# Ogeon/pyrite

Measured on AMD Instinct MI355X. Metric: Msamples/sec, higher is better.
Workload: dtype f32; 1 GPU; C3: c3_mesh_in_box, 1920x1080, 1024 spp; bounces=8, light_samples=4, spectrum_samples=10, spectrum_bins=64, tile_size=32, triangles=819212, spheres=0, parallelism=one launch on one GPU, film_weight_check=ok

## Files before the change

### pyrite_amd/csrc/api.cpp

```cpp
#include <hip/hip_runtime.h>

#include <algorithm>
#include <chrono>
#include <cmath>
#include <cstdlib>
#include <cstring>
#include <memory>
#include <new>
#include <string>
#include <vector>

#include "api_internal.h"
#include "bvh.h"
#include "bvh_device.h"
#include "device_scene.h"
#include "kernels/refit_launch.h"
#include "program_regs.h"

using namespace pyr;

namespace {

thread_local std::string g_error;
int fail(int code, const std::string& message) {
// ... 277 lines not shown
        if (!closed) return false;
    }
    chain.assign(outer_first.rbegin(), outer_first.rend());
    for (uint32_t reg : chain)
        if (reg >= PYR_MAX_NUMBER_REGISTERS) return false;
    hit = lambda = p;
    hit.first_instr = (uint32_t)instrs.size();
    hit.num_instrs = (uint32_t)hit_list.size();
    hit.output_reg = chain[0];
    instrs.insert(instrs.end(), hit_list.begin(), hit_list.end());
    lambda.first_instr = (uint32_t)instrs.size();
    lambda.num_instrs = (uint32_t)lambda_list.size();
    lambda.output_reg = instrs[(size_t)lambda_writer].output;
    instrs.insert(instrs.end(), lambda_list.begin(), lambda_list.end());
    return true;
}

}

struct PyrScene {
    int device = 0;
    int num_cus = 0;
    DevScene dev{};
    PyrBvhInfo info{};
    PyrBuildInfo build_info{};
    std::unique_ptr<pyr::BuiltBvh> digest_source;
    DeviceBuffer wide_nodes, wide_pair_nodes, pair_prims, nodes, prims, tri_shade, spheres, sphere_material, planes, plane_material, lamps, materials, components, programs, instrs, spectra,
        spectrum_data, rgb_basis, counters, tri_tex, sphere_tex_scale, plane_frames, textures, texture_data;
    PyrCounters last_counters{};
    bool have_counters = false;
    PyrProgramInfo program_info{};
    uint32_t* tail_count = nullptr;
    DeviceBuffer tape;
    DeviceBuffer tape_overflow;
    struct Geometry {
        std::vector<float> tri_positions, tri_normals, tri_uvs, tri_frames, spheres, sphere_tex_scale;
        std::vector<uint32_t> tri_material, sphere_material;
        std::vector<PyrLamp> lamps;
        bool has_uvs = false, has_frames = false, has_tex_scale = false;
        uint32_t num_triangles = 0, num_spheres = 0;
        PyrSceneDesc view() const {
            PyrSceneDesc d{};
            d.num_triangles = num_triangles, d.num_spheres = num_spheres, d.num_lamps = (uint32_t)lamps.size();
            d.tri_positions = tri_positions.data(), d.tri_normals = tri_normals.data(), d.tri_material = tri_material.data();
            d.tri_uvs = has_uvs ? tri_uvs.data() : nullptr, d.tri_frames = has_frames ? tri_frames.data() : nullptr;
            d.spheres = spheres.data(), d.sphere_material = sphere_material.data();
            d.sphere_tex_scale = has_tex_scale ? sphere_tex_scale.data() : nullptr;
            d.lamps = lamps.data();
            return d;
        }
    } geometry;
    void keep_geometry(const PyrSceneDesc* d) {
        Geometry& g = geometry;
        const size_t nt = d->num_triangles, ns = d->num_spheres;
        g.num_triangles = d->num_triangles, g.num_spheres = d->num_spheres;
        g.tri_positions.assign(d->tri_positions, d->tri_positions + (nt ? 9 * nt : 0));
        g.tri_normals.assign(d->tri_normals, d->tri_normals + (nt ? 9 * nt : 0));
        g.tri_material.assign(d->tri_material, d->tri_material + nt);
        g.has_uvs = d->tri_uvs != nullptr, g.has_frames = d->tri_frames != nullptr, g.has_tex_scale = d->sphere_tex_scale != nullptr;
        if (g.has_uvs) g.tri_uvs.assign(d->tri_uvs, d->tri_uvs + 6 * nt);
        if (g.has_frames) g.tri_frames.assign(d->tri_frames, d->tri_frames + 12 * nt);
        g.spheres.assign(d->spheres, d->spheres + (ns ? 4 * ns : 0));
        g.sphere_material.assign(d->sphere_material, d->sphere_material + ns);
        if (g.has_tex_scale) g.sphere_tex_scale.assign(d->sphere_tex_scale, d->sphere_tex_scale + 2 * ns);
        g.lamps.assign(d->lamps, d->lamps + d->num_lamps);
    }
// ... 513 lines not shown
    const uint32_t rows = p->film_row_count ? p->film_row_count : film->height;
    return (uint64_t)rows * film->width * film->bins;
}

int check_render_args(PyrScene* scene, const PyrCamera* camera, const PyrFilmDesc* film, const PyrRenderParams* p, const void* film_ptr) {
    if (!scene || !camera || !film || !p || !film_ptr) return fail(PYR_ERR_INVALID_ARGUMENT, "null argument");
    if (film->width == 0 || film->height == 0 || film->bins == 0 || p->tile_size == 0 || p->spectrum_samples == 0)
        return fail(PYR_ERR_INVALID_ARGUMENT, "zero-sized parameter");
    if (!(film->wl_width > 0.0f)) return fail(PYR_ERR_INVALID_ARGUMENT, "empty wavelength span");
    uint32_t rows = p->film_row_count ? p->film_row_count : film->height;
    if ((uint64_t)p->film_row_begin + rows > film->height) return fail(PYR_ERR_INVALID_ARGUMENT, "film window exceeds the image");
    if (p->spectrum_samples > 64) return fail(PYR_ERR_UNSUPPORTED, "spectrum_samples > 64");
    if ((uint64_t)film->width * film->height >= 0xFFFFFFFFull) return fail(PYR_ERR_UNSUPPORTED, "image too large: 2^32 pixels or more");
    if (p->film_layout == PYR_FILM_TILE_BLOCKS) {
        const uint64_t tiles = (uint64_t)((film->width + p->tile_size - 1) / p->tile_size) * ((film->height + p->tile_size - 1) / p->tile_size);
        if (tiles * (p->tile_size + 2ull) * (p->tile_size + 2ull) >= 0xFFFFFFFFull) return fail(PYR_ERR_UNSUPPORTED, "image too large for a film of tile blocks");
    }
    if (p->film_layout > PYR_FILM_TILE_BLOCKS) return fail(PYR_ERR_INVALID_ARGUMENT, "unknown film layout");
    if (p->film_layout == PYR_FILM_TILE_BLOCKS && (p->film_row_begin || p->film_row_count))
        return fail(PYR_ERR_INVALID_ARGUMENT, "a film of tile blocks has no row window");
    return PYR_OK;
}


int reserve_tape(PyrScene* scene, RenderLaunch& L, hipStream_t stream) {
    const size_t bytes = (size_t)L.tape_lanes * L.tape_max_ops * sizeof(unsigned long long);
    if (bytes > scene->tape.bytes) {
        HIP_TRY(hipStreamSynchronize(stream));
        scene->tape.release();
        int rc = scene->tape.alloc(bytes);
        if (rc != PYR_OK) return rc;
    }
    L.tape = (unsigned long long*)scene->tape.ptr;
    if (!scene->tape_overflow.ptr) {
        int rc = scene->tape_overflow.alloc(sizeof(uint32_t));
        if (rc != PYR_OK) return rc;
        HIP_TRY(hipMemsetAsync(scene->tape_overflow.ptr, 0, sizeof(uint32_t), stream));
    }
    L.tape_overflow = (uint32_t*)scene->tape_overflow.ptr;
    return PYR_OK;
}

void choose_schedule(const PyrScene* scene, RenderLaunch& L) {
    const char* e = std::getenv("PYRITE_SCHEDULER");
    if (e && std::string(e) == "sm")
        L.scheduler = 1;
    else if (e && std::string(e) == "sync")
        L.scheduler = 0;
    else
        L.scheduler = scene_is_lds_resident(scene->dev) && scene->dev.needs_interpreter == 0 ? 0u : 1u;
    if (L.scheduler == 0 && scene->dev.needs_interpreter != 0) L.scheduler = 1;
    const char* lanes = std::getenv("PYRITE_SM_LANES");
    const char* steps = std::getenv("PYRITE_SM_STEPS");
    L.sm_phase_lanes = lanes && *lanes ? (uint32_t)std::strtoul(lanes, nullptr, 10) : (scene->dev.needs_interpreter != 0 ? 32u : 16u);
    L.sm_trav_steps = steps && *steps ? (uint32_t)std::strtoul(steps, nullptr, 10) : 8u;
    const char* expose = std::getenv("PYRITE_SM_EXPOSE_LANES");
    L.sm_expose_lanes = expose && *expose ? (uint32_t)std::strtoul(expose, nullptr, 10) : L.sm_phase_lanes;
}

int render_batches(PyrScene* scene, RenderLaunch L, bool count, hipStream_t stream) {
    if (L.chunk_end == L.chunk_begin) return PYR_OK;
    choose_schedule(scene, L);
    if (L.scheduler != 0 && (scene->dev.needs_interpreter == 0 || uses_hit_tape(scene->dev, L))) {
        L.tape_lanes = tape_lanes_bound(scene->num_cus);
        L.tape_max_ops = tape_ops_bound(scene->dev, L);
        int rc = reserve_tape(scene, L, stream);
// ... 1350 lines not shown
```

### pyrite_amd/csrc/device_scene.h

```cpp
#pragma once
#include <cstddef>
#include <cstdint>

#include "../../include/pyrite_gpu.h"

namespace pyr {

struct DevPrim {
    float a[4], b[4], c[4];
};

struct DevPrimPair {
    float q[5][4];
};

struct DevTriShade {
    float n1[4], n2[4], n3[4];
};

struct DevTriTex {
    float uv12[4], uv3[4], f1[4], f2[4], f3[4];
};

struct DevTexture {
// ... 86 lines not shown
constexpr uint32_t tape_row(uint32_t slot) { return slot + (slot >= kTapeOneRow ? 1u : 0u); }
constexpr uint32_t tape_rgb_row(uint32_t n_spectral) { return n_spectral + 3u <= kTapeOneRow ? n_spectral : (n_spectral >= kTapeOneRow ? n_spectral + 1u : kTapeValueRows); }
constexpr uint32_t tape_rows_needed(uint32_t n_spectral, bool rgb) {
    return (rgb ? tape_rgb_row(n_spectral) + 3u : (n_spectral == 0u ? 0u : tape_row(n_spectral - 1u) + 1u)) > kTapeValueRows
               ? (rgb ? tape_rgb_row(n_spectral) + 3u : tape_row(n_spectral - 1u) + 1u)
               : kTapeValueRows;
}

constexpr uint32_t kMaxStackDepth = 64;

struct RenderLaunch {
    PyrCamera camera;
    PyrFilmDesc film;
    uint32_t bounces, light_samples, spectrum_samples, tile_size, pixel_samples;
    uint32_t tiles_x, tiles_y;
    uint32_t tile_begin, tile_stride, tile_count;
    uint32_t chunks_per_tile;
    uint32_t chunk_begin, chunk_end;
    uint32_t film_layout;
    uint32_t film_row_begin, film_row_count;
    uint64_t seed;
    float grains_per_wavelength;
    PyrGrain* film_out;
    unsigned long long* counters;
    uint32_t scheduler;
    uint32_t sm_phase_lanes, sm_trav_steps;
    uint32_t sm_expose_lanes;
    uint32_t stack_lds;
    unsigned long long* tape;
    uint32_t tape_lanes, tape_max_ops;
    uint32_t* tape_overflow;
    uint32_t tape_programs_lds;
    uint32_t sample_begin;
};

constexpr uint32_t kFeedSegments = 8, kFeedCursorStride = 64;
constexpr size_t kFeedBytes = (size_t)kFeedSegments * kFeedCursorStride * sizeof(uint32_t);

struct IntersectLaunch {
    const float* rays;
    PyrHit* hits;
    uint32_t n;
    unsigned long long* counters;
    uint32_t* next;
    uint32_t num_cus;
    uint32_t reserve;
    uint32_t stack_lds;
};

struct DevelopLaunch {
    PyrFilmDesc film;
    const PyrGrain* grains;
    float step_size, xyz_scale;
    uint32_t sample_count;
    const float* filter;
    const float* white_div;
    const float* white_mul;
    const float* xyz_table;
    uint32_t xyz_count;
    float xyz_min, xyz_max;
    uint8_t* rgb_out;
    const PyrGrain* grains_b;
};
int launch_develop(const DevelopLaunch& launch, void* stream);

constexpr uint32_t kWaveDevelopMaxBins = 255;
bool develop_wave_serves(const DevelopLaunch& launch);
// ... 83 lines not shown
```

### pyrite_amd/csrc/kernels.hip

```cpp
#ifndef PYRITE_KERNELS_HIP
#define PYRITE_KERNELS_HIP
#include <hip/hip_runtime.h>

#include <algorithm>
#include <cstdint>
#include <cstdlib>
#include <string>
#include <type_traits>

#include "device_scene.h"
#include "exact_math.h"

#ifdef PYR_WIDE_VM
#define PYR_VM_NUMBERS PYR_WIDE_NUMBER_REGISTERS
#define PYR_VM_VECTORS PYR_WIDE_VECTOR_REGISTERS
#define PYR_VM_RGBS PYR_WIDE_RGB_REGISTERS
#else
#define PYR_VM_NUMBERS PYR_MAX_NUMBER_REGISTERS
#define PYR_VM_VECTORS PYR_MAX_VECTOR_REGISTERS
#define PYR_VM_RGBS PYR_MAX_RGB_REGISTERS
#endif
static_assert((PYR_VM_NUMBERS & (PYR_VM_NUMBERS - 1)) == 0 && (PYR_VM_VECTORS & (PYR_VM_VECTORS - 1)) == 0 && (PYR_VM_RGBS & (PYR_VM_RGBS - 1)) == 0,
              "the interpreter masks register indices: its files are powers of two");

// ... 753 lines not shown
    float from_x, from_y, size_x, size_y;
};
DEV TileArea to_view_area(uint32_t x, uint32_t y, uint32_t w, uint32_t h, uint32_t width, uint32_t height) {
    float iw = (float)width, ih = (float)height;
    float half_max = __fmul_rn(fmaxf(iw, ih), 0.5f);
    TileArea a;
    a.from_x = __fdiv_rn(__fadd_rn((float)x, -__fmul_rn(iw, 0.5f)), half_max);
    a.from_y = __fdiv_rn(__fadd_rn((float)y, -__fmul_rn(ih, 0.5f)), half_max);
    a.size_x = __fdiv_rn((float)w, half_max);
    a.size_y = __fdiv_rn((float)h, half_max);
    return a;
}
DEV f3 transform_point(const float* m, f3 p) {
    float x = m[0] * p.x + m[4] * p.y + m[8] * p.z + m[12];
    float y = m[1] * p.x + m[5] * p.y + m[9] * p.z + m[13];
    float z = m[2] * p.x + m[6] * p.y + m[10] * p.z + m[14];
    float w = m[3] * p.x + m[7] * p.y + m[11] * p.z + m[15];
    float inv = 1.0f / w;
    return mk(x * inv, y * inv, z * inv);
}
DEV f3 transform_vector(const float* m, f3 v) {
    return mk(m[0] * v.x + m[4] * v.y + m[8] * v.z, m[1] * v.x + m[5] * v.y + m[9] * v.z, m[2] * v.x + m[6] * v.y + m[10] * v.z);
}
DEV uint32_t f32_as_index(float f) { return f > 0.0f ? (f >= 4294967040.0f ? 0xFFFFFFFFu : (uint32_t)f) : 0u; }

struct Spectral {
    float* base;
    uint32_t s;
    DEV float& wl(uint32_t k) { return base[(0 * s + k) * BLOCK]; }
    DEV float& bright(uint32_t k) { return base[(1 * s + k) * BLOCK]; }
    DEV float& refl(uint32_t k) { return base[(2 * s + k) * BLOCK]; }
};

DEV void surface_at(const DevScene& S, const Hit& hit, f3 o, f3 d, f3& position, f3& normal, uint32_t& material) {
    const uint32_t kind = hit.shape >> 30, index = hit.shape & 0x3FFFFFFFu;
    if (kind == PYR_SHAPE_TRIANGLE) {
        const float4* sh = reinterpret_cast<const float4*>(S.tri_shade) + 3 * (size_t)index;
        const float4 a = sh[0], b = sh[1], c = sh[2];
        float w = 1.0f - (hit.u + hit.v);
        normal = normalize(mk(a.x, a.y, a.z) * w + mk(b.x, b.y, b.z) * hit.u + mk(c.x, c.y, c.z) * hit.v);
        material = __float_as_uint(a.w);
        position = o + d * hit.t;
    } else if (kind == PYR_SHAPE_SPHERE) {
        const float4 sp = reinterpret_cast<const float4*>(S.spheres)[index];
        float dist;
        sphere_test(mk(sp.x, sp.y, sp.z), sp.w, o, d, dist, position);
        normal = normalize(position - mk(sp.x, sp.y, sp.z));
        material = S.sphere_material[index];
    } else {
        const float* pl = S.planes + 8 * index;
        float dist;
        plane_test(ld3(pl), ld3(pl + 3), o, d, dist, position);
        normal = ld3(pl + 3);
        material = S.plane_material[index];
    }
}

struct Quat {
    float s, x, y, z;
};
DEV Quat quat_scale(Quat q, float f) { return Quat{q.s * f, q.x * f, q.y * f, q.z * f}; }
DEV Quat quat_add(Quat a, Quat b) { return Quat{a.s + b.s, a.x + b.x, a.y + b.y, a.z + b.z}; }
DEV Quat quat_normalize(Quat q) {
    float m = sqrt32(q.s * q.s + q.x * q.x + q.y * q.y + q.z * q.z);
    return quat_scale(q, 1.0f / m);
}
// ... 259 lines not shown
DEV void expose_grain(const RenderLaunch& L, uint32_t pixel, float wavelength, float brightness, Counters& cnt) {
    if (pixel == PIXEL_NONE) return;
    uint32_t grain = f32_as_index(__fmul_rn(__fsub_rn(wavelength, L.film.wl_start), L.grains_per_wavelength));
    grain = grain < L.film.bins - 1 ? grain : L.film.bins - 1;
    float* g = reinterpret_cast<float*>(L.film_out + ((size_t)pixel * L.film.bins + grain));
    atomicAdd(g, brightness);
    atomicAdd(g + 1, 1.0f);
    if (COUNT) cnt.exposures++;
}

struct Path {
    Rng rng;
    uint32_t pixel;
    f3 o, d;
    float wl, bright, refl;
    uint32_t bounce, events;
    bool use_additional, sample_light;
};

struct SceneView {
    const float4* nodes;
    const float4* prims;
    bool wide = false;
    const float4* pairs = nullptr;
};
DEV SceneView wide_or_binary_view(const DevScene& S);
template <typename T>
DEV const T* own_scalar(const T* p) {
    unsigned long long in = (unsigned long long)p, out;
    asm volatile("s_mov_b64 %0, %1" : "=s"(out) : "s"(in));
    return reinterpret_cast<const T*>(out);
}

DEV SceneView wide_or_binary_view(const DevScene& S) {
    SceneView v{reinterpret_cast<const float4*>(S.nodes), reinterpret_cast<const float4*>(S.prims), false, nullptr};
    if (S.wide_nodes != nullptr) {
        v.nodes = reinterpret_cast<const float4*>(S.wide_nodes);
        v.wide = true;
    }
    return v;
}

template <bool LDS_SCENE>
DEV SceneView stage_scene(const DevScene& S, float* lds, uint32_t lds_floats_before, bool resumable = false) {
    SceneView v{reinterpret_cast<const float4*>(S.nodes), reinterpret_cast<const float4*>(S.prims)};
    if (!LDS_SCENE && resumable && S.wide_nodes != nullptr) {
        v.nodes = reinterpret_cast<const float4*>(S.wide_nodes);
        v.wide = true;
    }
    if (!LDS_SCENE && resumable && S.wide_nodes != nullptr && S.pair_prims != nullptr) {
        v.nodes = reinterpret_cast<const float4*>(S.wide_pair_nodes);
        v.pairs = reinterpret_cast<const float4*>(S.pair_prims);
    }
    if constexpr (!LDS_SCENE) {
        v.nodes = own_scalar(v.nodes);
        v.prims = own_scalar(v.prims);
        v.pairs = own_scalar(v.pairs);
    }
    if constexpr (LDS_SCENE) {
        float4* staged = reinterpret_cast<float4*>(lds + lds_floats_before);
        const uint32_t node_vecs = S.num_nodes * 4, prim_vecs = S.num_prims * 3;
        for (uint32_t i = threadIdx.x; i < node_vecs; i += BLOCK) staged[i] = v.nodes[i];
        for (uint32_t i = threadIdx.x; i < prim_vecs; i += BLOCK) staged[node_vecs + i] = v.prims[i];
        __syncthreads();
        v.nodes = staged;
        v.prims = staged + node_vecs;
    }
    return v;
}

template <int TABLES, bool COPY = true>
DEV DevScene stage_tables(const DevScene& S, float* lds, uint32_t lds_floats_before) {
    DevScene local = S;
    if (TABLES == 1 || (TABLES == -1 && S.lds_table_floats != 0)) {
        float* dst = lds + lds_floats_before;
        auto stage = [&](const void* src, uint32_t floats) {
            const float* from = reinterpret_cast<const float*>(src);
            if (COPY)
                for (uint32_t i = threadIdx.x; i < floats; i += BLOCK) dst[i] = from[i];
            float* at = dst;
            dst += floats;
            return at;
        };
        local.spectra = reinterpret_cast<const PyrSpectrum*>(stage(S.spectra, S.num_spectra * (uint32_t)(sizeof(PyrSpectrum) / sizeof(float))));
        local.spectrum_data = stage(S.spectrum_data, S.num_spectrum_floats);
        local.materials = reinterpret_cast<const PyrMaterial*>(stage(S.materials, S.num_materials * (uint32_t)(sizeof(PyrMaterial) / sizeof(float))));
        local.components = reinterpret_cast<const PyrComponent*>(stage(S.components, S.num_components * (uint32_t)(sizeof(PyrComponent) / sizeof(float))));
        local.programs = reinterpret_cast<const DevProgram*>(stage(S.programs, S.num_programs * (uint32_t)(sizeof(DevProgram) / sizeof(float))));
        local.lamps = reinterpret_cast<const DevLamp*>(stage(S.lamps, S.num_lamps * (uint32_t)(sizeof(DevLamp) / sizeof(float))));
        if (COPY) __syncthreads();
    }
    return local;
}

template <bool COMPANION_STATE = true>
DEV void start_sample(const RenderLaunch& L, uint32_t tile, uint64_t iteration, const TileArea& area, Path& p, Spectral& spec) {
    const uint32_t SS = L.spectrum_samples;
    p.rng = rng_seed(L.seed, tile, iteration);
    const float px = __fadd_rn(area.from_x, __fmul_rn(area.size_x, rng_f32(p.rng)));
    const float py = __fadd_rn(area.from_y, __fmul_rn(area.size_y, rng_f32(p.rng)));
    p.pixel = film_pixel(L, tile, px, py);
    {
        float focus_x = px / L.camera.view_plane * L.camera.focus_distance;
        float focus_y = py / L.camera.view_plane * L.camera.focus_distance;
        f3 target = mk(focus_x, -focus_y, -L.camera.focus_distance);
        f3 origin = mk(0, 0, 0), direction = target;
        if (L.camera.aperture > 0.0f) {
            float sqrt_r = sqrt32(L.camera.aperture * rng_f32(p.rng));
            float psi = PI_F * 2.0f * rng_f32(p.rng);
            origin = mk(sqrt_r * cos32(psi), sqrt_r * sin32(psi), 0.0f);
            direction = target - origin;
        }
        p.o = transform_point(L.camera.cam_to_world, origin);
        p.d = transform_vector(L.camera.cam_to_world, normalize(direction));
    }
    {
        float step_size = L.film.wl_width / (float)SS;
        float from = L.film.wl_start;
        for (uint32_t k = 0; k < SS; ++k) {
            float to = __fadd_rn(from, step_size);
            spec.wl(k) = rng_range_f32(p.rng, from, to);
            from = to;
        }
        uint32_t hero = rng_range_usize(p.rng, SS);
        p.wl = spec.wl(hero);
        spec.wl(hero) = spec.wl(SS - 1);
        if constexpr (COMPANION_STATE)
            for (uint32_t k = 0; k + 1 < SS; ++k) {
                spec.bright(k) = 0.0f;
// ... 275 lines not shown
    for (uint32_t chunk = L.chunk_begin + wave; chunk < L.chunk_end; chunk += total_waves) {
        uint32_t tile;
        uint64_t iteration;
        TileArea area;
        if (!locate_chunk(L, chunk, lane, tile, iteration, area)) continue;
        Path p{};
        start_sample(launch_from_kernarg(L), tile, iteration, area, p, spec);
        if (COUNT) cnt.samples++;
        SLAP(sp, 0);
        while (p.bounce < L.bounces) {
            const bool ended = bounce_step<COUNT>(S, launch_from_kernarg(L), view, p, spec, stack, cnt, sp);
            p.bounce++;
            if (ended) break;
        }
        SLAP(sp, 6);
        SYNC_PRIO(SYNC_PRIO_E);
        finish_path<COUNT>(launch_from_kernarg(L), p, spec, cnt);
        SLAP(sp, 7);
    }
#ifdef PYR_PHASE_PROFILE
    if (lane == 0)
        for (int i = 0; i < 8; ++i) atomicAdd(&g_phase_prof[i], sp.section[i]);
#endif
    flush_counters<COUNT>(cnt, L.counters);
}

#ifdef PYR_PHASE_PROFILE
#define PROF_DECL unsigned long long prof_c[4] = {0, 0, 0, 0}, prof_l[4] = {0, 0, 0, 0}, prof_n[4] = {0, 0, 0, 0}
#define PROF_BEGIN(ph, cond) const unsigned long long prof_t0_##ph = clock64(); prof_l[ph] += __popcll(ballot64(cond)); prof_n[ph]++
#define PROF_END(ph) prof_c[ph] += clock64() - prof_t0_##ph
#define PROF_LANES(ph, cond) prof_l[ph] += __popcll(ballot64(cond)); prof_n[ph]++
#define PROF_NOW() clock64()
#define PROF_EXTRA(idx, cycles) if ((threadIdx.x & 63u) == 0) atomicAdd(&g_phase_prof[idx], (unsigned long long)(cycles))
#define PROF_FLUSH()                                                                                  \
    if ((threadIdx.x & 63u) == 0)                                                                     \
        for (int i = 0; i < 4; ++i) {                                                                 \
            atomicAdd(&g_phase_prof[i], prof_c[i]);                                                   \
            atomicAdd(&g_phase_prof[4 + i], prof_l[i]);                                               \
            atomicAdd(&g_phase_prof[8 + i], prof_n[i]);                                               \
        }
#else
#define PROF_DECL
#define PROF_BEGIN(ph, cond)
#define PROF_END(ph)
#define PROF_LANES(ph, cond)
#define PROF_NOW() 0ull
#define PROF_EXTRA(idx, cycles)
#define PROF_FLUSH()
#endif

enum Stage : uint32_t { ST_NEW = 0, ST_TRAV = 1, ST_SHADE = 2, ST_NEE = 3, ST_EXPOSE = 4, ST_DONE = 5 };

struct Trav {
    f3 o, d, inv;
    uint32_t nx = 0, ny = 0, nz = 0;
    float limit, closest;
    int node, sp;
    uint32_t shape;
    float u, v;
    bool shadow, blocked;
};

DEV void trav_ray_signs(Trav& t) {
    t.nx = (__float_as_uint(t.d.x) >> 31) * 48u;
    t.ny = (__float_as_uint(t.d.y) >> 31) * 48u;
    t.nz = (__float_as_uint(t.d.z) >> 31) * 48u;
}
DEV float shadow_cutoff(float limit, float margin) { return __builtin_amdgcn_sqrtf(limit * margin + 1.0e-3f); }
DEV void trav_restart(Trav& t, float shadow_margin) {
    if (t.shadow) t.closest = shadow_cutoff(t.limit, shadow_margin);
    t.blocked = false;
    t.node = 0;
    t.sp = 0;
}

template <bool COUNT>
DEV bool trav_begin(const DevScene& S, Trav& t, f3 o, f3 d, bool shadow, float limit, Counters& cnt) {
    t.o = o;
    t.d = d;
    t.shadow = shadow;
    t.blocked = false;
    t.limit = shadow ? limit : -PYR_INF;
    t.closest = PYR_INF;
    t.shape = PYR_HIT_NONE;
    t.u = t.v = 0.0f;
    for (uint32_t i = 0; i < S.num_planes; ++i) {
        const float* pl = S.planes + 8 * i;
        float dist;
        f3 point;
        if (COUNT) cnt.plane_tests++;
        if (plane_test(ld3(pl), ld3(pl + 3), o, d, dist, point)) {
            if (shadow) {
                if (dist > DIST_EPSILON && dist * dist < limit) {
                    t.blocked = true;
                    return true;
                }
            } else if (dist > DIST_EPSILON && dist < t.closest) {
                t.closest = dist;
                t.shape = ((uint32_t)PYR_SHAPE_PLANE << 30) | i;
            }
        }
    }
    trav_restart(t, S.shadow_margin);
    return false;
}

typedef __attribute__((address_space(3))) int lds_int;
struct TravStack {
    lds_int* lds;
    int lds_entries;
    int* deep;
    DEV void push(int sp, int value) {
        if (sp < lds_entries)
            lds[sp * BLOCK] = value;
        else
            deep[sp - lds_entries] = value;
    }
    DEV int pop(int sp) const { return sp < lds_entries ? lds[sp * BLOCK] : deep[sp - lds_entries]; }
};

template <bool COUNT, bool SIGNED = false>
DEV void wide_node_children(const float4 lx, const float4 ly, const float4 lz, const float4 hx, const float4 hy, const float4 hz, const float4 ch, const Trav& t,
                            Counters& cnt, float (&e)[4], int (&c)[4]) {
    const f2v ix = {t.inv.x, t.inv.x}, iy = {t.inv.y, t.inv.y}, iz = {t.inv.z, t.inv.z};
    const float ox = -(t.o.x * t.inv.x), oy = -(t.o.y * t.inv.y), oz = -(t.o.z * t.inv.z);
    const f2v nox = {ox, ox}, noy = {oy, oy}, noz = {oz, oz};
    c[0] = __float_as_int(ch.x), c[1] = __float_as_int(ch.y), c[2] = __float_as_int(ch.z), c[3] = __float_as_int(ch.w);
    {
        const f2v alx = __builtin_elementwise_fma((f2v){lx.x, lx.y}, ix, nox), ahx = __builtin_elementwise_fma((f2v){hx.x, hx.y}, ix, nox);
        const f2v aly = __builtin_elementwise_fma((f2v){ly.x, ly.y}, iy, noy), ahy = __builtin_elementwise_fma((f2v){hy.x, hy.y}, iy, noy);
        const f2v alz = __builtin_elementwise_fma((f2v){lz.x, lz.y}, iz, noz), ahz = __builtin_elementwise_fma((f2v){hz.x, hz.y}, iz, noz);
        const f2v blx = __builtin_elementwise_fma((f2v){lx.z, lx.w}, ix, nox), bhx = __builtin_elementwise_fma((f2v){hx.z, hx.w}, ix, nox);
        const f2v bly = __builtin_elementwise_fma((f2v){ly.z, ly.w}, iy, noy), bhy = __builtin_elementwise_fma((f2v){hy.z, hy.w}, iy, noy);
        const f2v blz = __builtin_elementwise_fma((f2v){lz.z, lz.w}, iz, noz), bhz = __builtin_elementwise_fma((f2v){hz.z, hz.w}, iz, noz);
        const float tl[4][3] = {{alx.x, aly.x, alz.x}, {alx.y, aly.y, alz.y}, {blx.x, bly.x, blz.x}, {blx.y, bly.y, blz.y}};
        const float th[4][3] = {{ahx.x, ahy.x, ahz.x}, {ahx.y, ahy.y, ahz.y}, {bhx.x, bhy.x, bhz.x}, {bhx.y, bhy.y, bhz.y}};
        for (int k = 0; k < 4; ++k) {
            const float tmin = SIGNED ? fmaxf(fmaxf(tl[k][0], tl[k][1]), tl[k][2])
                                      : fmaxf(fmaxf(fminf(tl[k][0], th[k][0]), fminf(tl[k][1], th[k][1])), fminf(tl[k][2], th[k][2]));
            const float tmax = SIGNED ? fminf(fminf(th[k][0], th[k][1]), th[k][2])
// ... 274 lines not shown
struct Walker {
    uint32_t stage = ST_NEW;
    uint32_t n_ops = 0;
    uint32_t tape_column = 0;
    const uint32_t* tape_prepared = nullptr;
    DEV void tape_push(const RenderLaunch& L, uint32_t kind, uint32_t program, float s, bool hero_only = false) {
        if (n_ops < L.tape_max_ops) {
            uint32_t word = (kind << 30) | (hero_only ? TAPE_HERO_ONLY : 0u) | (program & TAPE_PROGRAM_MASK);
            if (tape_prepared != nullptr) {
                uint32_t slot = kTapeOneSlot;
                if (kind != TAPE_SCALE) {
                    const uint32_t* e = tape_prepared + 8 * program;
                    if (e[0] == 0u)
                        s = __uint_as_float(e[1]) * s;
                    else
                        slot = e[7];
                }
                word = (kind == TAPE_ADD ? TAPE_EAGER_ADD : 0u) | (hero_only ? TAPE_HERO_ONLY : 0u) | (slot << TAPE_EAGER_SLOT_SHIFT);
            }
            L.tape[tape_index(n_ops, L.tape_lanes, tape_column)] = (unsigned long long)word | ((unsigned long long)__float_as_uint(s) << 32);
        } else {
            *L.tape_overflow = 1u;
        }
        n_ops++;
    }
    DEV void tape_push_raw(const RenderLaunch& L, uint32_t word, float s) {
        if (n_ops < L.tape_max_ops)
            L.tape[tape_index(n_ops, L.tape_lanes, tape_column)] = (unsigned long long)word | ((unsigned long long)__float_as_uint(s) << 32);
        else
            *L.tape_overflow = 1u;
        n_ops++;
    }
    uint32_t rgb_slot = 0;
    uint32_t chunk = 0;
    Path p{};
    Trav t{};
    f3 b_position = mk(0, 0, 0), b_normal = mk(0, 0, 0), b_out = mk(0, 0, 0);
    bool b_flip = false;
    DEV f3 b_nff() const { return b_flip ? -b_normal : b_normal; }
    bool b_has_brdf = false;
    uint32_t nee_lamp = 0, nee_i = 0;
    DEV static float nee_probability(const DevScene& S, const RenderLaunch& L) {
        const float lamp_probability = 1.0f / (float)S.num_lamps;
        return 1.0f / ((float)L.light_samples * 2.0f * PI_F * lamp_probability);
    }
    bool ls_pending = false, ls_physical = false;
    uint32_t ls_material = 0, ls_color = 0;
    f3 ls_normal = mk(0, 0, 0);
    float ls_scale = 0.0f;
    float ls_tx = 0.0f, ls_ty = 0.0f;

    enum : uint32_t { CONTRIB_NONE = 0, CONTRIB_MUL = 1, CONTRIB_ADD = 2 };
    uint32_t c_kind = CONTRIB_NONE, c_color = 0;
    int c_probability = -1;
    float c_cp = 1.0f, c_outer = 1.0f, c_scale = 1.0f;
    bool c_use_outer = false, c_companions = false, c_has_scale = false;
    f3 c_normal = mk(0, 0, 0), c_incident = mk(0, 0, 0);
    float c_tx = 0.0f, c_ty = 0.0f;
    DEV void contribution(uint32_t kind, uint32_t color, int probability, float cp, bool use_outer, float outer, bool companions, f3 normal, f3 incident, float tx,
                          float ty) {
        c_kind = kind, c_color = color, c_probability = probability, c_cp = cp, c_use_outer = use_outer, c_outer = outer, c_companions = companions;
        c_normal = normal, c_incident = incident, c_tx = tx, c_ty = ty;
    }
    DEV void contribution_clear() {
        c_kind = CONTRIB_NONE, c_color = 0u, c_probability = -1;
        c_cp = 1.0f, c_outer = 1.0f, c_scale = 1.0f;
        c_use_outer = false, c_companions = false, c_has_scale = false;
// ... 109 lines not shown
    }

    DEV void finish_bounce(const DevScene& S, const RenderLaunch& L, Spectral& spec, Counters& cnt) {
        const uint32_t n_add = L.spectrum_samples - 1;
        if (b_has_brdf) {
            const float brdf = 2.0f * fabsf(dot(b_out, b_normal));
            if constexpr (TAPE && !INTERP) {
                tape_push(L, TAPE_SCALE, 0u, brdf);
            } else if constexpr (INTERP) {
                c_scale = brdf, c_has_scale = true;
            } else {
                p.refl *= brdf;
                if (p.use_additional) {
                    for (uint32_t k = 0; k < n_add; ++k) spec.refl(k) *= brdf;
                }
            }
        }
        p.o = b_position;
        p.d = b_out;
        p.bounce++;
        if (p.bounce >= L.bounces) {
            stage = ST_EXPOSE;
        } else {
            if (COUNT) cnt.extension_rays++;
            stage = trav_begin<COUNT>(S, t, p.o, p.d, false, 0.0f, cnt) ? ST_SHADE : ST_TRAV;
        }
    }

    DEV void expose_and_restart(const DevScene& S, const RenderLaunch& L, Spectral& spec, Counters& cnt, uint32_t lane, uint32_t total_waves) {
        if (stage == ST_EXPOSE) {
            if constexpr (!TAPE) finish_path<COUNT>(L, p, spec, cnt);
            stage = ST_NEW;
        }
        if (stage == ST_NEW) {
            stage = ST_DONE;
            while (chunk < L.chunk_end) {
                uint32_t tile;
                uint64_t iteration;
                TileArea area;
                const bool ok = locate_chunk(L, chunk, lane, tile, iteration, area);
                chunk += total_waves;
                if (ok) {
                    start_sample<!TAPE>(L, tile, iteration, area, p, spec);
                    n_ops = 0;
                    if (COUNT) cnt.samples++;
                    if (L.bounces == 0) {
                        stage = ST_EXPOSE;
                    } else {
                        if (COUNT) cnt.extension_rays++;
                        stage = trav_begin<COUNT>(S, t, p.o, p.d, false, 0.0f, cnt) ? ST_SHADE : ST_TRAV;
                    }
                    break;
                }
            }
        }
    }

    DEV void shade(const DevScene& S, const RenderLaunch& L, Spectral& spec, Counters& cnt) {
        if (stage != ST_SHADE) return;
        const uint32_t n_add = L.spectrum_samples - 1;
        const f3 ray_o = t.o, ray_d = t.d;
        if (t.shape == PYR_HIT_NONE) {
            uint32_t color = S.sky_program;
            if (p.sample_light) {
                for (uint32_t i = 0; i < S.num_lamps; ++i) {
                    const DevLamp& l = S.lamps[i];
                    if (l.kind == PYR_LAMP_DIRECTIONAL && dot(ld3(l.v), ray_d) >= l.width) {
                        color = l.color_program;
                        break;
                    }
                }
            }
            if constexpr (TAPE && !INTERP) {
                tape_push(L, TAPE_ADD, color, 1.0f);
            } else if constexpr (INTERP) {
                contribution(CONTRIB_ADD, color, -1, 1.0f, false, 1.0f, p.use_additional, -ray_d, ray_d, 0.0f, 0.0f);
            } else {
                const Prepared q_prog = prepare_program<INTERP>(S, color);
                VmInput in{p.wl, -ray_d, ray_d};
                p.bright += eval_prepared<INTERP>(S, q_prog, in) * 1.0f * p.refl;
                if (p.use_additional)
                    for (uint32_t k = 0; k < n_add; ++k) {
                        in.wavelength = spec.wl(k);
                        spec.bright(k) += eval_prepared<INTERP>(S, q_prog, in) * 1.0f * spec.refl(k);
                    }
            }
            stage = ST_EXPOSE;
// ... 442 lines not shown
    for (uint32_t i = 0; i < L.tape_programs_lds; ++i) n_spectral += (reads_spectrum(i) && first_alike(i) == i) ? 1u : 0u;
    for (uint32_t i = threadIdx.x; i < L.tape_programs_lds; i += BLOCK) {
        const Prepared q = prepare_program<false>(S, i);
        const bool spectral = reads_spectrum(i);
        const uint32_t representative = spectral ? first_alike(i) : i;
        const uint32_t slot = spectral ? slot_of(representative) : 0u;
        uint32_t* e = prepared_lds + 8 * i;
        e[0] = q.mode, e[1] = __float_as_uint(q.c), e[2] = q.sp.format, e[3] = __float_as_uint(q.sp.min), e[4] = __float_as_uint(q.sp.max);
        e[5] = q.sp.offset, e[6] = q.sp.count, e[7] = tape_row(slot);
        if (spectral && representative == i && slot < kTapeMaxValueRows - 1u) prepared_lds[8 * L.tape_programs_lds + slot] = i;
    }
    __syncthreads();
    eager = L.tape_programs_lds != 0 && tape_rows_needed(n_spectral, S0.rgb_records != 0) <= S0.tape_value_rows && (n_spectral != 0 || S0.hit_tape != 0);
    return eager ? n_spectral : 0u;
}

#ifndef PYR_SM_WAVES_INTERP
#define PYR_SM_WAVES_INTERP 3
#endif
constexpr int sm_waves(bool interp) { return interp ? PYR_SM_WAVES_INTERP : PYR_SM_WAVES; }
template <bool COUNT, bool INTERP, bool LDS_SCENE, bool LDS_TABLES, bool HIT_TAPE = false, bool PRODUCT = false>
__global__ __launch_bounds__(BLOCK, sm_waves(INTERP)) void render_kernel_sm(DevScene S0, RenderLaunch L) {
    extern __shared__ float lds[];
    static_assert(INTERP || !HIT_TAPE, "HIT_TAPE is a form of the interpreter build");
    static_assert(HIT_TAPE || !PRODUCT, "PRODUCT is a form of the hit tape (device_scene.h TapeForm)");
    constexpr bool TAPE = !INTERP || HIT_TAPE;
    const uint32_t SS = L.spectrum_samples;
    Spectral spec{lds + threadIdx.x, SS};
    const uint32_t spectral_rows = TAPE ? SS + 1 + S0.tape_value_rows : 3 * SS;
    TravStack stack;
    int deep_levels[LDS_SCENE ? 1 : kMaxStackDepth];
    stack.deep = deep_levels;
    stack.lds = (lds_int*)(reinterpret_cast<int*>(lds + spectral_rows * BLOCK) + threadIdx.x);
    stack.lds_entries = (int)L.stack_lds;
    Counters cnt{};
    const uint32_t lds_base_floats = (spectral_rows + L.stack_lds) * BLOCK;
    const SceneView view = stage_scene<LDS_SCENE>(S0, lds, lds_base_floats, true);
    const DevScene S = stage_tables<LDS_TABLES ? 1 : 0>(S0, lds, lds_base_floats + (LDS_SCENE ? (S0.num_nodes * 16 + S0.num_prims * 12) : 0));

    const uint32_t lane = threadIdx.x & 63u;
    const uint32_t waves_per_block = BLOCK / 64;
    const uint32_t total_waves = gridDim.x * waves_per_block;
    const int phase_lanes = (int)L.sm_phase_lanes, trav_steps = (int)L.sm_trav_steps;
    const int expose_lanes = TAPE ? (int)L.sm_expose_lanes : phase_lanes;
    Walker<COUNT, INTERP, TAPE, PRODUCT> w;
    w.chunk = L.chunk_begin + blockIdx.x * waves_per_block + (threadIdx.x >> 6);
    w.tape_prepared = nullptr;
    uint32_t* wave_list = reinterpret_cast<uint32_t*>(lds + SS * BLOCK) + (threadIdx.x & ~63u);
    uint32_t* prepared_lds = reinterpret_cast<uint32_t*>(lds + lds_base_floats + (LDS_SCENE ? (S0.num_nodes * 16 + S0.num_prims * 12) : 0) + (LDS_TABLES ? S0.lds_table_floats : 0));
    uint32_t n_spectral = 0;
    bool eager = false;
    float* spectral_values = lds + (SS + 1) * BLOCK + threadIdx.x;
    if constexpr (TAPE) {
        spectral_values[kTapeOneSlot * BLOCK] = 1.0f;
        n_spectral = prepare_tape_tables(S0, S, L, prepared_lds, eager);
        if (eager) w.tape_prepared = prepared_lds;
        w.rgb_slot = tape_rgb_row(n_spectral);
        w.tape_column = blockIdx.x * BLOCK + threadIdx.x;
        if (HIT_TAPE && !eager) *L.tape_overflow = 1u;
    }

    auto scene_view = [&](const RenderLaunch& Lp) {
        if (LDS_SCENE || INTERP) return S;
        const uint32_t rows = (TAPE ? Lp.spectrum_samples + 1 + S0.tape_value_rows : 3 * Lp.spectrum_samples) + Lp.stack_lds;
        return stage_tables<LDS_TABLES ? 1 : 0, false>(scene_from_kernarg(S0), lds, rows * BLOCK);
    };
    PROF_DECL;
    for (;;) {
        int nT = __popcll(ballot64(w.stage == ST_TRAV));
        int nS = __popcll(ballot64(w.stage == ST_SHADE));
        int nN = __popcll(ballot64(w.stage == ST_NEE));
        int nE = __popcll(ballot64(w.stage == ST_EXPOSE || w.stage == ST_NEW));
        if (max(max(nT, nS), max(nN, nE)) == 0) break;

        if (nE >= expose_lanes || nE == max(max(nT, nS), max(nN, nE))) {
            PHASE_PRIO(PYR_PRIO_E);
            PROF_BEGIN(0, w.stage == ST_EXPOSE || w.stage == ST_NEW);
            const RenderLaunch& Lp = launch_from_kernarg(L);
            const DevScene Sp = scene_view(Lp);
            if constexpr (TAPE)
                replay_tapes<COUNT, HIT_TAPE, PRODUCT>(Sp, Lp, w.stage == ST_EXPOSE, w.n_ops, w.tape_column, w.p, lds, threadIdx.x, wave_list, prepared_lds, spectral_values, n_spectral,
                                              HIT_TAPE ? eager : n_spectral != 0, cnt);
            w.expose_and_restart(Sp, Lp, spec, cnt, lane, total_waves);
            PROF_END(0);
            nT = __popcll(ballot64(w.stage == ST_TRAV));
            nS = __popcll(ballot64(w.stage == ST_SHADE));
            nE = 0;
        }
        if (nS >= phase_lanes || nS == max(max(nT, nS), max(nN, nE))) {
            PHASE_PRIO(PYR_PRIO_S);
            PROF_BEGIN(1, w.stage == ST_SHADE);
            const RenderLaunch& Lp = launch_from_kernarg(L);
            w.shade(scene_view(Lp), Lp, spec, cnt);
            PROF_END(1);
            nT = __popcll(ballot64(w.stage == ST_TRAV));
            nN = __popcll(ballot64(w.stage == ST_NEE));
            nE = __popcll(ballot64(w.stage == ST_EXPOSE || w.stage == ST_NEW));
            nS = 0;
        }
        if (nN >= phase_lanes || nN == max(max(nT, nS), max(nN, nE))) {
            PHASE_PRIO(PYR_PRIO_N);
            PROF_BEGIN(2, w.stage == ST_NEE);
            const RenderLaunch& Lp = launch_from_kernarg(L);
            w.next_event(scene_view(Lp), Lp, spec, cnt);
            PROF_END(2);
            nT = __popcll(ballot64(w.stage == ST_TRAV));
            nN = __popcll(ballot64(w.stage == ST_NEE));
            nE = __popcll(ballot64(w.stage == ST_EXPOSE || w.stage == ST_NEW));
        }
        if constexpr (INTERP) {
            const unsigned long long pending = ballot64(w.c_kind != 0u || w.c_has_scale);
            if (pending != 0ull) {
                [[maybe_unused]] const unsigned long long t_c0 = PROF_NOW();
                PROF_EXTRA(13, __popcll(pending));
                PROF_EXTRA(14, 1);
                const RenderLaunch& Lp = launch_from_kernarg(L);
                if constexpr (HIT_TAPE)
                    w.tape_pending(scene_view(Lp), Lp);
                else
                    w.contribute_pending(scene_view(Lp), Lp, spec);
                PROF_EXTRA(12, PROF_NOW() - t_c0);
            }
            w.contribution_clear();
        }
        if (nT >= phase_lanes || nT == max(max(nT, nS), max(nN, nE))) {
#ifdef PYR_PHASE_PROFILE
            const unsigned long long prof_t0_3 = clock64();
#endif
            PHASE_PRIO(PYR_PRIO_T);
            w.t.inv = box_reciprocal(w.t.d);
            trav_ray_signs(w.t);
            if (!LDS_SCENE && view.wide && view.pairs != nullptr) {
                for (int step = 0; step < trav_steps; ++step) {
                    PROF_LANES(3, w.stage == ST_TRAV);
                    if (trav_step_lean<COUNT>(view, w.t, stack, cnt, w.stage == ST_TRAV)) w.stage = w.t.shadow ? ST_NEE : ST_SHADE;
                }
            } else {
                for (int step = 0; step < trav_steps; ++step) {
                    PROF_LANES(3, w.stage == ST_TRAV);
                    if (trav_step_voted<COUNT, !LDS_SCENE>(view, w.t, stack, cnt, w.stage == ST_TRAV)) w.stage = w.t.shadow ? ST_NEE : ST_SHADE;
                }
            }
            PROF_END(3);
        }
    }
    PROF_FLUSH();
    flush_counters<COUNT>(cnt, L.counters);
}


struct WorkFeed {
    uint32_t next = 0, end = 0;
    uint32_t segment = 0, visited = 0;
    bool drained = false;
};
DEV uint32_t feed_segment_begin(uint32_t n, uint32_t segment) { return (uint32_t)(((uint64_t)n * segment / kFeedSegments) & ~63ull); }
DEV uint32_t feed_segment_end(uint32_t n, uint32_t segment) { return segment + 1 == kFeedSegments ? n : feed_segment_begin(n, segment + 1); }
DEV void feed_reserve(WorkFeed& f, uint32_t* cursors, uint32_t n, uint32_t reserve, uint32_t lane) {
    while (f.next == f.end && !f.drained) {
        const uint32_t begin = feed_segment_begin(n, f.segment), end = feed_segment_end(n, f.segment);
        uint32_t base = 0;
        if (lane == 0) base = atomicAdd(&cursors[f.segment * kFeedCursorStride], reserve);
        base = __shfl(base, 0, 64);
        if (base < end - begin) {
            f.next = begin + base;
            f.end = begin + min(base + reserve, end - begin);
        } else if (++f.visited == kFeedSegments) {
            f.drained = true;
        } else {
            f.segment = (f.segment + 1) % kFeedSegments;
        }
    }
}

#ifndef PYR_INTERSECT_PAIRS
#define PYR_INTERSECT_PAIRS 1
#endif
#ifndef PYR_INTERSECT_WAVES
#define PYR_INTERSECT_WAVES 5
// ... 75 lines not shown
```

### pyrite_amd/csrc/kernels/main.hip

```cpp
#include "../kernels.hip"

namespace pyr {

namespace {
thread_local std::string g_kernel_error;
}
const char* kernels_last_error() { return g_kernel_error.c_str(); }

__global__ __launch_bounds__(BLOCK) void develop_kernel(DevelopLaunch D) {
    const size_t pixels = (size_t)D.film.width * D.film.height;
    const uint32_t bins = D.film.bins;
    const float min = D.film.wl_start, max = D.film.wl_start + D.film.wl_width;
    for (size_t px = (size_t)blockIdx.x * BLOCK + threadIdx.x; px < pixels; px += (size_t)gridDim.x * BLOCK) {
        uint8_t out[3] = {0, 0, 0};
        if ((px + 1) * bins < pixels * bins) {
            const PyrGrain* g = D.grains + px * bins;
            auto xyz_get = [&](int channel, float w) {
                const float* d = D.xyz_table;
                const uint32_t n = D.xyz_count;
                if (w <= D.xyz_min) return d[channel];
                if (w >= D.xyz_max) return d[3 * (n - 1) + channel];
                float normalized = (w - D.xyz_min) / (D.xyz_max - D.xyz_min);
                float fi = normalized * ((float)n - 1.0f);
                float fmin_ = truncf(fi);
// ... 199 lines not shown
    const size_t lds = render_lds_bytes(scene, launch);
    if (lds > 160 * 1024) {
        g_kernel_error = "spectrum_samples + BVH depth need more than 160 KB of LDS per workgroup";
        return PYR_ERR_UNSUPPORTED;
    }
    const uint32_t chunks = launch.chunk_end - launch.chunk_begin;
    if (chunks == 0) return PYR_OK;
    RenderKernel kernel = pick_kernel(launch.scheduler == 1, with_counters, scene.needs_interpreter != 0, scene_fits_lds(scene), scene.lds_table_floats != 0,
                                      launch.scheduler == 1 && uses_hit_tape(scene, launch), scene.product_records != 0, wide_vm);
    if (kernel == nullptr) {
        g_kernel_error = "a program of this scene needs the wide interpreter build, which this one-unit build of the kernels does not hold";
        return PYR_ERR_UNSUPPORTED;
    }
    hipError_t err = hipFuncSetAttribute(reinterpret_cast<const void*>(kernel), hipFuncAttributeMaxDynamicSharedMemorySize, (int)lds);
    if (err != hipSuccess) {
        g_kernel_error = std::string("hipFuncSetAttribute: ") + hipGetErrorString(err);
        return PYR_ERR_DEVICE;
    }
    hipFuncAttributes attr{};
    int blocks_per_cu = 4;
    if (hipFuncGetAttributes(&attr, reinterpret_cast<const void*>(kernel)) == hipSuccess && attr.numRegs > 0) {
        int regs = ((attr.numRegs + 7) / 8) * 8;
        blocks_per_cu = std::min(8, 512 / regs);
    }
    blocks_per_cu = std::max(1, std::min<int>(blocks_per_cu, (int)((160 * 1024) / std::max<size_t>(lds, 1))));
    uint32_t grid = (uint32_t)num_cus * (uint32_t)blocks_per_cu;
    const uint32_t path_waves = BLOCK / 64;
    uint32_t blocks_needed = (chunks + path_waves - 1) / path_waves;
    if (grid > blocks_needed) grid = blocks_needed;
    if (uses_tape(scene, launch) && (launch.tape == nullptr || (size_t)grid * BLOCK > launch.tape_lanes || launch.tape_max_ops < tape_ops_bound(scene, launch))) {
        g_kernel_error = "the spectral tape is missing or too small for this launch";
        return PYR_ERR_INVALID_ARGUMENT;
    }
    if (const char* cut = std::getenv("PYRITE_TEST_TAPE_OPS"))
        if (uses_tape(scene, launch) && *cut) launch.tape_max_ops = std::min<uint32_t>(launch.tape_max_ops, (uint32_t)std::strtoul(cut, nullptr, 10));
    hipLaunchKernelGGL(kernel, dim3(grid), dim3(BLOCK), lds, (hipStream_t)stream, scene, launch);
    err = hipGetLastError();
    if (err != hipSuccess) {
        g_kernel_error = std::string("render kernel launch: ") + hipGetErrorString(err);
        return PYR_ERR_DEVICE;
    }
    return PYR_OK;
}

int launch_intersect(const DevScene& scene, const IntersectLaunch& launch, bool with_counters, void* stream) {
    if (launch.n == 0) return PYR_OK;
    if (scene.stack_depth > kMaxStackDepth) {
        g_kernel_error = "BVH deeper than kMaxStackDepth";
        return PYR_ERR_UNSUPPORTED;
    }
    const uint32_t stack_lds = short_stack_levels(scene, 0, 8);
    const size_t lds = (size_t)stack_lds * BLOCK * sizeof(int);
    auto kernel = with_counters ? intersect_kernel<true> : intersect_kernel<false>;
    hipError_t err = hipFuncSetAttribute(reinterpret_cast<const void*>(kernel), hipFuncAttributeMaxDynamicSharedMemorySize, (int)lds);
    if (err != hipSuccess) {
        g_kernel_error = std::string("hipFuncSetAttribute: ") + hipGetErrorString(err);
        return PYR_ERR_DEVICE;
    }
    int blocks_per_cu = std::max(1, std::min<int>(8, (int)((160 * 1024) / std::max<size_t>(lds, 1))));
    uint32_t grid = (uint32_t)launch.num_cus * (uint32_t)blocks_per_cu;
    uint32_t needed = (launch.n + BLOCK - 1) / BLOCK;
    if (grid > needed) grid = needed;
    IntersectLaunch sized = launch;
    sized.stack_lds = stack_lds;
    const uint32_t waves = grid * (BLOCK / 64);
    sized.reserve = std::max<uint32_t>(64, std::min<uint32_t>(2048, (launch.n / std::max<uint32_t>(waves * 4, 1)) & ~63u));
// ... 11 lines not shown
```

Before: 631.8 Msamples/s.

## Queue precomputed sample starts per wave to batch restart work across lanes

```diff
diff --git a/pyrite_amd/csrc/api.cpp b/pyrite_amd/csrc/api.cpp
--- a/pyrite_amd/csrc/api.cpp
+++ b/pyrite_amd/csrc/api.cpp
@@ -333,6 +333,7 @@
     PyrProgramInfo program_info{};
     uint32_t* tail_count = nullptr;
     DeviceBuffer tape;
+    DeviceBuffer start_queue;
     DeviceBuffer tape_overflow;
     struct Geometry {
         std::vector<float> tri_positions, tri_normals, tri_uvs, tri_frames, spheres, sphere_tex_scale;
@@ -912,6 +913,17 @@
         if (rc != PYR_OK) return rc;
     }
     L.tape = (unsigned long long*)scene->tape.ptr;
+    if (scene->dev.needs_interpreter == 0) {
+        L.start_queue_stride = start_queue_words(L.spectrum_samples) * kStartQueueEntries;
+        const size_t queue_bytes = (size_t)(L.tape_lanes / 64u) * L.start_queue_stride * sizeof(uint32_t);
+        if (queue_bytes > scene->start_queue.bytes) {
+            HIP_TRY(hipStreamSynchronize(stream));
+            scene->start_queue.release();
+            int rc = scene->start_queue.alloc(queue_bytes);
+            if (rc != PYR_OK) return rc;
+        }
+        L.start_queue = (uint32_t*)scene->start_queue.ptr;
+    }
     if (!scene->tape_overflow.ptr) {
         int rc = scene->tape_overflow.alloc(sizeof(uint32_t));
         if (rc != PYR_OK) return rc;
diff --git a/pyrite_amd/csrc/device_scene.h b/pyrite_amd/csrc/device_scene.h
--- a/pyrite_amd/csrc/device_scene.h
+++ b/pyrite_amd/csrc/device_scene.h
@@ -142,7 +142,15 @@
     uint32_t* tape_overflow;
     uint32_t tape_programs_lds;
     uint32_t sample_begin;
-};
+    uint32_t* start_queue;
+    uint32_t start_queue_stride;
+};
+
+#ifndef PYR_SAMPLE_QUEUE
+#define PYR_SAMPLE_QUEUE 1
+#endif
+constexpr uint32_t kStartQueueEntries = 128, kStartQueueFixedWords = 11;
+constexpr uint32_t start_queue_words(uint32_t spectrum_samples) { return kStartQueueFixedWords + spectrum_samples; }
 
 constexpr uint32_t kFeedSegments = 8, kFeedCursorStride = 64;
 constexpr size_t kFeedBytes = (size_t)kFeedSegments * kFeedCursorStride * sizeof(uint32_t);
diff --git a/pyrite_amd/csrc/kernels.hip b/pyrite_amd/csrc/kernels.hip
--- a/pyrite_amd/csrc/kernels.hip
+++ b/pyrite_amd/csrc/kernels.hip
@@ -809,6 +809,13 @@
     DEV float& refl(uint32_t k) { return base[(2 * s + k) * BLOCK]; }
 };
 
+typedef __attribute__((address_space(1))) uint32_t global_u32;
+typedef __attribute__((address_space(1))) float global_f32;
+struct StartQueueRows {
+    global_f32* base;
+    DEV global_f32& wl(uint32_t k) { return base[k * kStartQueueEntries]; }
+};
+
 DEV void surface_at(const DevScene& S, const Hit& hit, f3 o, f3 d, f3& position, f3& normal, uint32_t& material) {
     const uint32_t kind = hit.shape >> 30, index = hit.shape & 0x3FFFFFFFu;
     if (kind == PYR_SHAPE_TRIANGLE) {
@@ -1134,6 +1141,12 @@
     return reinterpret_cast<const T*>(out);
 }
 
+DEV uint32_t own_scalar(uint32_t v) {
+    uint32_t out;
+    asm volatile("s_mov_b32 %0, %1" : "=s"(out) : "s"(v));
+    return out;
+}
+
 DEV SceneView wide_or_binary_view(const DevScene& S) {
     SceneView v{reinterpret_cast<const float4*>(S.nodes), reinterpret_cast<const float4*>(S.prims), false, nullptr};
     if (S.wide_nodes != nullptr) {
@@ -1195,8 +1208,8 @@
     return local;
 }
 
-template <bool COMPANION_STATE = true>
-DEV void start_sample(const RenderLaunch& L, uint32_t tile, uint64_t iteration, const TileArea& area, Path& p, Spectral& spec) {
+template <bool COMPANION_STATE = true, class ROWS = Spectral>
+DEV void start_sample(const RenderLaunch& L, uint32_t tile, uint64_t iteration, const TileArea& area, Path& p, ROWS& spec) {
     const uint32_t SS = L.spectrum_samples;
     p.rng = rng_seed(L.seed, tile, iteration);
     const float px = __fadd_rn(area.from_x, __fmul_rn(area.size_x, rng_f32(p.rng)));
@@ -1538,6 +1551,7 @@
 #define PROF_LANES(ph, cond) prof_l[ph] += __popcll(ballot64(cond)); prof_n[ph]++
 #define PROF_NOW() clock64()
 #define PROF_EXTRA(idx, cycles) if ((threadIdx.x & 63u) == 0) atomicAdd(&g_phase_prof[idx], (unsigned long long)(cycles))
+#define PROF_ADD(acc, v) (acc) += (v)
 #define PROF_FLUSH()                                                                                  \
     if ((threadIdx.x & 63u) == 0)                                                                     \
         for (int i = 0; i < 4; ++i) {                                                                 \
@@ -1552,6 +1566,7 @@
 #define PROF_LANES(ph, cond)
 #define PROF_NOW() 0ull
 #define PROF_EXTRA(idx, cycles)
+#define PROF_ADD(acc, v)
 #define PROF_FLUSH()
 #endif
 
@@ -1612,6 +1627,7 @@
 }
 
 typedef __attribute__((address_space(3))) int lds_int;
+typedef __attribute__((address_space(3))) uint32_t lds_u32;
 struct TravStack {
     lds_int* lds;
     int lds_entries;
@@ -1952,7 +1968,12 @@
         n_ops++;
     }
     uint32_t rgb_slot = 0;
+    static constexpr bool QUEUE = PYR_SAMPLE_QUEUE != 0 && TAPE && !INTERP;
     uint32_t chunk = 0;
+    uint32_t q_state = 0;
+#ifdef PYR_PHASE_PROFILE
+    unsigned long long prof_start[4] = {0, 0, 0, 0};
+#endif
     Path p{};
     Trav t{};
     f3 b_position = mk(0, 0, 0), b_normal = mk(0, 0, 0), b_out = mk(0, 0, 0);
@@ -2128,16 +2149,64 @@
             if constexpr (!TAPE) finish_path<COUNT>(L, p, spec, cnt);
             stage = ST_NEW;
         }
-        if (stage == ST_NEW) {
-            stage = ST_DONE;
-            while (chunk < L.chunk_end) {
+        if constexpr (QUEUE) {
+            [[maybe_unused]] const unsigned long long prof_q0 = PROF_NOW();
+            const unsigned long long starting = ballot64(stage == ST_NEW);
+            uint32_t wanted = (uint32_t)__popcll(starting);
+            asm volatile("" : "+v"(wanted));
+            const unsigned long long below = (1ull << lane) - 1ull;
+            global_u32* slab = (global_u32*)(L.start_queue + (size_t)(tape_column >> 6) * L.start_queue_stride);
+            const uint32_t q_head = q_state & (kStartQueueEntries - 1u);
+            uint32_t q_count = q_state >> 8;
+            bool filled = false;
+            while (q_count < wanted && chunk < L.chunk_end) {
                 uint32_t tile;
                 uint64_t iteration;
                 TileArea area;
                 const bool ok = locate_chunk(L, chunk, lane, tile, iteration, area);
                 chunk += total_waves;
+                const unsigned long long exist = ballot64(ok);
+                const uint32_t at = q_head + q_count + (uint32_t)__popcll(exist & below);
+                q_count += (uint32_t)__popcll(exist);
                 if (ok) {
-                    start_sample<!TAPE>(L, tile, iteration, area, p, spec);
+                    global_u32* e = slab + (at & (kStartQueueEntries - 1u));
+                    Path s;
+                    StartQueueRows rows{(global_f32*)(e + kStartQueueFixedWords * kStartQueueEntries)};
+                    start_sample<false>(L, tile, iteration, area, s, rows);
+                    rows.wl(L.spectrum_samples - 1u) = s.wl;
+                    e[0 * kStartQueueEntries] = s.rng.x, e[1 * kStartQueueEntries] = s.rng.y, e[2 * kStartQueueEntries] = s.rng.z, e[3 * kStartQueueEntries] = s.rng.w;
+                    e[4 * kStartQueueEntries] = s.pixel;
+                    e[5 * kStartQueueEntries] = __float_as_uint(s.o.x), e[6 * kStartQueueEntries] = __float_as_uint(s.o.y), e[7 * kStartQueueEntries] = __float_as_uint(s.o.z);
+                    e[8 * kStartQueueEntries] = __float_as_uint(s.d.x), e[9 * kStartQueueEntries] = __float_as_uint(s.d.y), e[10 * kStartQueueEntries] = __float_as_uint(s.d.z);
+                }
+                filled = true;
+            }
+            if (filled) __builtin_amdgcn_fence(__ATOMIC_RELEASE, "workgroup");
+            [[maybe_unused]] const unsigned long long prof_q1 = PROF_NOW();
+            PROF_ADD(prof_start[0], prof_q1 - prof_q0);
+            PROF_ADD(prof_start[1], filled ? 1 : 0);
+            __builtin_amdgcn_fence(__ATOMIC_ACQUIRE, "workgroup");
+            if (stage == ST_NEW) {
+                const uint32_t rank = (uint32_t)__popcll(ballot64(stage == ST_NEW) & below);
+                stage = ST_DONE;
+                if (rank < q_count) {
+                    const global_u32* e = slab + ((q_head + rank) & (kStartQueueEntries - 1u));
+                    const uint32_t n_add = L.spectrum_samples - 1u;
+                    lds_u32* rows = (lds_u32*)(reinterpret_cast<uint32_t*>(spec.base) - lane);
+                    for (uint32_t k = 0; k < n_add; ++k)
+                        __builtin_amdgcn_global_load_lds(e + (kStartQueueFixedWords + k) * kStartQueueEntries, rows + k * BLOCK, 4, 0, 0);
+                    p.rng = Rng{e[0 * kStartQueueEntries], e[1 * kStartQueueEntries], e[2 * kStartQueueEntries], e[3 * kStartQueueEntries]};
+                    p.pixel = e[4 * kStartQueueEntries];
+                    p.o = mk(__uint_as_float(e[5 * kStartQueueEntries]), __uint_as_float(e[6 * kStartQueueEntries]), __uint_as_float(e[7 * kStartQueueEntries]));
+                    p.d = mk(__uint_as_float(e[8 * kStartQueueEntries]), __uint_as_float(e[9 * kStartQueueEntries]), __uint_as_float(e[10 * kStartQueueEntries]));
+                    p.wl = __uint_as_float(e[(kStartQueueFixedWords + n_add) * kStartQueueEntries]);
+                    asm volatile("s_waitcnt vmcnt(0)" ::: "memory");
+                    p.bright = 0.0f;
+                    p.refl = 1.0f;
+                    p.use_additional = true;
+                    p.sample_light = true;
+                    p.events = 0;
+                    p.bounce = 0;
                     n_ops = 0;
                     if (COUNT) cnt.samples++;
                     if (L.bounces == 0) {
@@ -2146,9 +2215,37 @@
                         if (COUNT) cnt.extension_rays++;
                         stage = trav_begin<COUNT>(S, t, p.o, p.d, false, 0.0f, cnt) ? ST_SHADE : ST_TRAV;
                     }
-                    break;
                 }
             }
+            const uint32_t popped = min(wanted, q_count);
+            q_state = ((q_head + popped) & (kStartQueueEntries - 1u)) | ((q_count - popped) << 8);
+            asm volatile("" : "+v"(q_state));
+            PROF_ADD(prof_start[2], PROF_NOW() - prof_q1);
+        } else {
+            [[maybe_unused]] const unsigned long long prof_q0 = PROF_NOW();
+            if (stage == ST_NEW) {
+                stage = ST_DONE;
+                while (chunk < L.chunk_end) {
+                    uint32_t tile;
+                    uint64_t iteration;
+                    TileArea area;
+                    const bool ok = locate_chunk(L, chunk, lane, tile, iteration, area);
+                    chunk += total_waves;
+                    if (ok) {
+                        start_sample<!TAPE>(L, tile, iteration, area, p, spec);
+                        n_ops = 0;
+                        if (COUNT) cnt.samples++;
+                        if (L.bounces == 0) {
+                            stage = ST_EXPOSE;
+                        } else {
+                            if (COUNT) cnt.extension_rays++;
+                            stage = trav_begin<COUNT>(S, t, p.o, p.d, false, 0.0f, cnt) ? ST_SHADE : ST_TRAV;
+                        }
+                        break;
+                    }
+                }
+            }
+            PROF_ADD(prof_start[0], PROF_NOW() - prof_q0);
         }
     }
 
@@ -2657,7 +2754,8 @@
     int deep_levels[LDS_SCENE ? 1 : kMaxStackDepth];
     stack.deep = deep_levels;
     stack.lds = (lds_int*)(reinterpret_cast<int*>(lds + spectral_rows * BLOCK) + threadIdx.x);
-    stack.lds_entries = (int)L.stack_lds;
+    constexpr bool QUEUE = Walker<COUNT, INTERP, TAPE, PRODUCT>::QUEUE;
+    stack.lds_entries = QUEUE ? (int)own_scalar(L.stack_lds) : (int)L.stack_lds;
     Counters cnt{};
     const uint32_t lds_base_floats = (spectral_rows + L.stack_lds) * BLOCK;
     const SceneView view = stage_scene<LDS_SCENE>(S0, lds, lds_base_floats, true);
@@ -2666,8 +2764,8 @@
     const uint32_t lane = threadIdx.x & 63u;
     const uint32_t waves_per_block = BLOCK / 64;
     const uint32_t total_waves = gridDim.x * waves_per_block;
-    const int phase_lanes = (int)L.sm_phase_lanes, trav_steps = (int)L.sm_trav_steps;
-    const int expose_lanes = TAPE ? (int)L.sm_expose_lanes : phase_lanes;
+    const int phase_lanes = QUEUE ? (int)own_scalar(L.sm_phase_lanes) : (int)L.sm_phase_lanes, trav_steps = QUEUE ? (int)own_scalar(L.sm_trav_steps) : (int)L.sm_trav_steps;
+    const int expose_lanes = TAPE ? (QUEUE ? (int)own_scalar(L.sm_expose_lanes) : (int)L.sm_expose_lanes) : phase_lanes;
     Walker<COUNT, INTERP, TAPE, PRODUCT> w;
     w.chunk = L.chunk_begin + blockIdx.x * waves_per_block + (threadIdx.x >> 6);
     w.tape_prepared = nullptr;
@@ -2703,9 +2801,12 @@
             PROF_BEGIN(0, w.stage == ST_EXPOSE || w.stage == ST_NEW);
             const RenderLaunch& Lp = launch_from_kernarg(L);
             const DevScene Sp = scene_view(Lp);
-            if constexpr (TAPE)
+            if constexpr (TAPE) {
+                [[maybe_unused]] const unsigned long long t_r0 = PROF_NOW();
                 replay_tapes<COUNT, HIT_TAPE, PRODUCT>(Sp, Lp, w.stage == ST_EXPOSE, w.n_ops, w.tape_column, w.p, lds, threadIdx.x, wave_list, prepared_lds, spectral_values, n_spectral,
                                               HIT_TAPE ? eager : n_spectral != 0, cnt);
+                PROF_ADD(w.prof_start[3], PROF_NOW() - t_r0);
+            }
             w.expose_and_restart(Sp, Lp, spec, cnt, lane, total_waves);
             PROF_END(0);
             nT = __popcll(ballot64(w.stage == ST_TRAV));
@@ -2770,6 +2871,10 @@
         }
     }
     PROF_FLUSH();
+#ifdef PYR_PHASE_PROFILE
+    if constexpr (!INTERP)
+        for (int i = 0; i < 4; ++i) PROF_EXTRA(12 + i, w.prof_start[i]);
+#endif
     flush_counters<COUNT>(cnt, L.counters);
 }
 
diff --git a/pyrite_amd/csrc/kernels/main.hip b/pyrite_amd/csrc/kernels/main.hip
--- a/pyrite_amd/csrc/kernels/main.hip
+++ b/pyrite_amd/csrc/kernels/main.hip
@@ -255,6 +255,11 @@
         g_kernel_error = "the spectral tape is missing or too small for this launch";
         return PYR_ERR_INVALID_ARGUMENT;
     }
+    if (PYR_SAMPLE_QUEUE != 0 && uses_tape(scene, launch) && scene.needs_interpreter == 0 &&
+        (launch.start_queue == nullptr || launch.start_queue_stride < start_queue_words(launch.spectrum_samples) * kStartQueueEntries)) {
+        g_kernel_error = "the queue of ready sample starts is missing or too small for this launch";
+        return PYR_ERR_INVALID_ARGUMENT;
+    }
     if (const char* cut = std::getenv("PYRITE_TEST_TAPE_OPS"))
         if (uses_tape(scene, launch) && *cut) launch.tape_max_ops = std::min<uint32_t>(launch.tape_max_ops, (uint32_t)std::strtoul(cut, nullptr, 10));
     hipLaunchKernelGGL(kernel, dim3(grid), dim3(BLOCK), lds, (hipStream_t)stream, scene, launch);
```

Result: faster. 657.0 Msamples/s, median of 6 (+4.0%).
